# roseDwayane/EyeGaze-Multimodal

Measured on AMD Instinct MI355X. Metric: train samples/sec (gaze+EEG windows), higher is better.
Workload: dtype bf16; 1 GPU; cfg3: BASELINE configs[2]/[3]: + bidirectional cross-stream attention fusion; batch_per_gpu=256, global_batch=256, C=8, T=1024, seq_len=65, d_model=256, layers=6, step=fwd(train,dropout)+bwd+allreduce+clip+AdamW, parallelism=dp1

## Files before the change

### eyegaze_multimodal_amd/_lib.py

```python
from __future__ import annotations

import ctypes as C
from pathlib import Path

_PKG = Path(__file__).resolve().parent
LIB_PATH = _PKG / "libeyegaze_hip.so"

EG_F32, EG_BF16, EG_F16 = 0, 1, 2
ACT_NONE, ACT_RELU, ACT_GELU = 0, 1, 2
ABI_VERSION = 5


class EgError(RuntimeError):
    pass


class RowMap(C.Structure):
    _fields_ = [("row_stride", C.c_int64), ("group_stride", C.c_int64), ("rows_per_group", C.c_int32), ("_pad", C.c_int32)]


def rowmap(row_stride: int, group_stride: int = 0, rows_per_group: int = 0) -> RowMap:
    return RowMap(int(row_stride), int(group_stride), int(rows_per_group), 0)


# ... 19 lines not shown

class FfnDesc(C.Structure):
    _fields_ = [("A", C.c_void_p), ("W1", C.c_void_p), ("W2", C.c_void_p), ("H", C.c_void_p), ("C", C.c_void_p),
                ("bias1", C.c_void_p), ("bias2", C.c_void_p), ("gate", C.c_void_p), ("gate_bits_out", C.c_void_p),
                ("gate_bits_in", C.c_void_p), ("residual", C.c_void_p),
                ("state", C.c_void_p),
                ("lda", C.c_int64), ("ldh", C.c_int64), ("ldc", C.c_int64), ("ldg", C.c_int64), ("ldr", C.c_int64),
                ("M", C.c_int32), ("F", C.c_int32), ("act1", C.c_int32), ("dtype", C.c_int32),
                ("drop_h_p", C.c_float), ("drop_c1_p", C.c_float), ("drop_c2_p", C.c_float),
                ("drop_h_site", C.c_uint32), ("drop_c1_site", C.c_uint32), ("drop_c2_site", C.c_uint32),
                ("gate_scale", C.c_float),
                ("ln_gamma", C.c_void_p), ("ln_beta", C.c_void_p), ("ln_out", C.c_void_p), ("ln_stats", C.c_void_p)]


class LnBwdProjDesc(C.Structure):
    _fields_ = [("dy", C.c_void_p), ("x", C.c_void_p), ("stats", C.c_void_p), ("gamma", C.c_void_p), ("W_frag", C.c_void_p),
                ("dx", C.c_void_p), ("dx_drop", C.c_void_p), ("dC", C.c_void_p), ("partial", C.c_void_p), ("state", C.c_void_p),
                ("M", C.c_int32), ("d_model", C.c_int32), ("dtype", C.c_int32), ("partial_capacity_blocks", C.c_int32),
                ("drop1_p", C.c_float), ("drop2_p", C.c_float), ("drop1_site", C.c_uint32), ("drop2_site", C.c_uint32)]


class AttnBlockDesc(C.Structure):
    _fields_ = [("x", C.c_void_p), ("wqkv_frag", C.c_void_p), ("wo_frag", C.c_void_p), ("bqkv", C.c_void_p), ("bo", C.c_void_p),
                ("qkv", C.c_void_p), ("ctx", C.c_void_p), ("lse", C.c_void_p), ("r1", C.c_void_p), ("state", C.c_void_p),
                ("NB", C.c_int32), ("S", C.c_int32), ("d_model", C.c_int32), ("num_heads", C.c_int32), ("dtype", C.c_int32),
                ("attn_drop_p", C.c_float), ("out_drop_p", C.c_float), ("attn_drop_site", C.c_uint32), ("out_drop_site", C.c_uint32),
                ("ln_gamma", C.c_void_p), ("ln_beta", C.c_void_p), ("ln_out", C.c_void_p), ("ln_stats", C.c_void_p)]


class PackEntry(C.Structure):
    _fields_ = [("src", C.c_uint64), ("dst", C.c_uint64), ("rows", C.c_int32), ("cols", C.c_int32), ("ldd", C.c_int32),
                ("mode", C.c_int32), ("blk0", C.c_int32), ("nblk", C.c_int32)]


class PackEntryEx(C.Structure):
    _fields_ = [("src", C.c_uint64), ("dst", C.c_uint64), ("rows", C.c_int32), ("cols", C.c_int32), ("ldd", C.c_int32),
                ("mode", C.c_int32), ("blk0", C.c_int32), ("nblk", C.c_int32), ("p0", C.c_int32), ("p1", C.c_int32),
                ("p2", C.c_int32), ("p3", C.c_int32), ("src_elems", C.c_int64), ("dst_elems", C.c_int64)]


class TNProblem(C.Structure):
    _fields_ = [("dY", C.c_uint64), ("X", C.c_uint64), ("partial", C.c_uint64), ("ldy", C.c_int64), ("ldx", C.c_int64),
                ("N", C.c_int32), ("K", C.c_int32), ("part_rows", C.c_int32), ("has_bias", C.c_int32), ("blk0", C.c_int32),
                ("_pad", C.c_int32)]


class ReduceEntry(C.Structure):
    _fields_ = [("partial", C.c_uint64), ("out", C.c_uint64), ("n", C.c_int64), ("stride", C.c_int64),
                ("splits", C.c_int32), ("blk0", C.c_int32)]


class GemmTNDesc(C.Structure):
    _fields_ = [("dY", C.c_void_p), ("X", C.c_void_p), ("partial", C.c_void_p), ("y", RowMap), ("x", RowMap),
                ("M", C.c_int32), ("N", C.c_int32), ("K", C.c_int32), ("splits", C.c_int32), ("dtype", C.c_int32),
                ("x_tile_stride", C.c_int64), ("part_rows", C.c_int32), ("has_bias", C.c_int32), ("tile", C.c_int32)]


_P, _I, _L, _F, _U = C.c_void_p, C.c_int, C.c_int64, C.c_float, C.c_uint32

SIGNATURES = {
    "eg_device_info": [C.POINTER(C.c_int), C.c_char_p, _I],
    "eg_window_pack": [_P, _P, _I, _I, _I, _I, _I, _I, _I, _P],
    "eg_pack_table": [_P, _I, _I, _I, _P],
    "eg_pack_table_ex_check": [_P, _I, _I, C.POINTER(C.c_int)],
    "eg_pack_table_ex": [_P, _I, _I, _I, _P],
    "eg_cast": [_P, _P, _L, _I, _P],
    "eg_transpose_cast": [_P, _P, _I, _I, _I, _I, _P],
    "eg_pack_conv_weight": [_P, _P, _I, _I, _I, _I, _I, _I, _P],
    "eg_pack_convT_weight": [_P, _P, _I, _I, _I, _I, _I, _P],
    "eg_gemm_nt": [C.POINTER(GemmDesc), _P],
    "eg_gemm_nt_route": [C.POINTER(GemmDesc)],
    "eg_ffn_chain": [C.POINTER(FfnDesc), _P],
    "eg_ln_bwd_proj": [C.POINTER(LnBwdProjDesc), _P],
    "eg_ln_bwd_proj_blocks": [_I],
    "eg_attn_block_fwd": [C.POINTER(AttnBlockDesc), _P],
    "eg_attn_block_ok": [_I, _I, _I, _I],
    "eg_gemm_tn": [C.POINTER(GemmTNDesc), _P],
    "eg_reduce_partials": [_P, _P, _L, _I, _L, _I, _P],
    "eg_gemm_tn_grouped": [_P, _I, _I, _I, _I, _I, _P],
    "eg_gemm_tn_grouped256": [_P, _I, _I, _I, _I, _I, _P],
    "eg_reduce_table": [_P, _I, _I, _P],
    "eg_unpack_conv_wgrad": [_P, _P, _I, _I, _I, _I, _I, _I, _P],
    "eg_colsum": [_P, RowMap, _I, _I, _P, _I, _I, _P],
    "eg_layernorm_fwd": [_P, _P, _P, _P, _P, _I, _I, _I, _P],
    "eg_layernorm_bwd": [_P, _P, _P, _P, _P, _P, _P, _I, _I, _I, _I, _I, _F, _U, _F, _U, _P, _P],
    "eg_attention_fwd": [_P, _P, _P, _I, _I, _I, _I, _I, _F, _U, _P, _P],
    "eg_attention_bwd": [_P, _P, _P, _P, _P, _I, _I, _I, _I, _I, _F, _U, _P, _P],
    "eg_window_normalize": [_P, _P, _P, _I, _I, _I, _I, _P],
    "eg_attention_probs": [_P, _P, _P, _I, _I, _I, _I, _I, _P],
    "eg_attention_long_fwd": [_P, _P, _P, _I, _I, _I, _I, _I, _F, _U, _P, _P],
    "eg_attention_long_bwd": [_P, _P, _P, _P, _P, _I, _I, _I, _I, _I, _F, _U, _P, _P, _L, _P],
    "eg_attention_long_probs": [_P, _P, _P, _I, _I, _I, _I, _I, _P],
    "eg_rows_bcast_f32": [_P, _P, _P, _I, _I, _I, _I, _I, _I, _I, _P],
    "eg_rows_copy": [_P, _I, _I, _I, _I, _I, _I, _I, _I, _P],
    "eg_pool_fuse_fwd": [_P, _P, _P, _P, _P, _P, _P, _I, _I, _I, _I, _I, _I, _I, _P],
    "eg_pool_fuse_bwd": [_P, _P, _P, _P, _P, _P, _P, _P, _I, _I, _I, _I, _I, _I, _I, _P],
    "eg_classifier_ce_fwd": [_P, _P, _P, _P, _P, _P, _P, _I, _I, _I, _I, _P],
    "eg_classifier_ce_bwd": [_P, _P, _P, _P, _P, _P, _P, _P, _P, _P, _I, _I, _I, _I, _F, _I, _P],
    "eg_batch_rowsum": [_P, _P, _I, _I, _I, _I, _I, _P],
    "eg_rows_gather_gate": [_P, _P, _P, RowMap, _I, _I, _I, _I, _I, _I, _F, _I, _P],
    "eg_heads_fwd": [_P, _P, _P, _P, _P, _P, _P, _P, _P, _P, _P, _P, _P, _P, _I, _I, _I, _F, _U, _P, _I, _P],
    "eg_classifier_ce_bwd_fused": [_P, _P, _P, _P, _P, _P, _P, _P, _P, _P, _I, _I, _I, _I, _F, _I, _P],
    "eg_heads_bwd_chain": [_P, _P, _P, _P, _P, _P, _P, _P, _I, _I, _I, _P],
    "eg_heads_bwd_pool": [_P, _P, _P, _P, _P, _P, _P, _P, _P, _P, _P, _I, _I, _I, _I, _I, _I, _I, _P],
    "eg_token_grad_tail": [_P, _P, _P, RowMap, _P, _P, _I, _I, _I, _I, _I, _F, _I, _P],
    "eg_grad_sqnorm": [_P, _L, _P, _I, _P],
    "eg_grad_accumulate": [_P, _P, _L, _I, _P, _I, _P],
    "eg_clip_coef": [_P, _I, _F, _P, _P],
    "eg_grad_sqnorm_clip": [_P, _L, _P, _I, _F, _P, _P, _P],
    "eg_adamw": [_P, _P, _P, _P, _L, _F, _F, _F, _F, _P, _P],
    "eg_fill_f32": [_P, _L, _F, _P],
    "eg_adamw_group": [_P, _P, _P, _P, _L, _F, _F, _F, _F, _F, _P, _P],
    "eg_set_step_state": [_P, _U, _U, _F, _F, _F, _F, _I, _F, _I, _P],
    "eg_scaler_update": [_P, _F, _F, _I, _P],
    "eg_aux_symmetry": [_P, _P, _P, _P, _P, _I, _I, _P],
    "eg_aux_infonce": [_P, _P, _P, _F, _P, _P, _P, _P, _P, _I, _I, _P],
    "eg_aux_supcon": [_P, _P, _F, _P, _P, _P, _I, _I, _P],
    "eg_fuzzy_gate_fwd": [_P, _P, _P, _P, _P, _I, _I, _I, _F, _F, _F, _P],
    "eg_fusion_loop_loss": [_P, _P, _P, _P, _P, _P, _P, _P, _P, _P, _I, _I, _I, _F, _F, _F, _F, _F, _F, _P, _P],
    "eg_fuzzy_gate_bwd": [_P, _P, _P, _P, _P, _P, _P, _P, _I, _I, _I, _F, _F, _F, _P],
    "eg_ibs_analytic": [_P, _P, _P, _P, _P, _I, _I, _F, _I, _P, _P, _I, _P],
    "eg_ibs_pairs": [_P, _P, _P, _P, _P, _I, _I, _I, _F, _I, _P, _P, _I, _P],
    "eg_ibs_scalar": [_P, _P, _P, _P, _I, _I, _I, _F, _I, _P, _P, _I, _I, _I, _I, _P],
    "eg_affine_grad": [_P, _P, _P, _I, _I, _I, _I, _P],
    "eg_ibs_inorm": [_P, _P, _P, _P, _P, _P, _I, _I, _I, _I, _I, _I, _P],
    "eg_gelu_fwd": [_P, _P, _L, _I, _F, _U, _P, _P],
    "eg_gelu_bwd": [_P, _P, _P, _L, _I, _F, _U, _P, _P],
    "eg_stft_logmag": [_P, _P, _P, _I, _I, _I, _I, _I, _P],
    "eg_spec_conv1_fwd": [_P, _P, _P, _P, _I, _I, _I, _I, _P],
    "eg_spec_conv1_bwd": [_P, _P, _P, _P, _P, _I, _I, _I, _I, _P],
    "eg_spec_avgpool_fwd": [_P, _P, _I, _I, _I, _I, _P],
    "eg_spec_avgpool_bwd": [_P, _P, _P, _I, _I, _I, _I, _P],
    "eg_pack_conv2d_weight": [_P, _P, _I, _I, _I, _I, _P],
    "eg_unpack_conv2d_wgrad": [_P, _P, _I, _I, _I, _P],
    "eg_conv2d_wgrad_flat": [_P, _P, _P, _P, _L, _L, _I, _I, _I, _P],
    "eg_conv2d_wgrad_flat_splits": [_L, _I],
    "eg_conv2d_flat": [_P, _P, _P, _P, _L, _L, _I, _I, _I, _I, _I, _I, _I, _P],
}
_lib = None


def lib() -> C.CDLL:
    global _lib
    if _lib is not None:
        return _lib
    if not LIB_PATH.exists():
        raise EgError(f"{LIB_PATH} is missing: build it with `python -m eyegaze_multimodal_amd.build` "
                      "(hipcc --offload-arch=gfx950).  There is no CPU fallback.")
    l = C.CDLL(str(LIB_PATH))
    l.eg_abi_version.restype = C.c_int
    if l.eg_abi_version() != ABI_VERSION:
        raise EgError(f"ABI mismatch: library {l.eg_abi_version()} vs binding {ABI_VERSION}")
    l.eg_last_error.restype = C.c_char_p
    for name, args in SIGNATURES.items():
        fn = getattr(l, name, None)
        if fn is None:
            continue
        fn.argtypes = args
        fn.restype = C.c_int
    _lib = l
    return l


def gate_bits_bytes(M: int, F: int) -> int:
    l = lib()
    l.eg_ffn_gate_bits_bytes.restype = C.c_int64
# ... 24 lines not shown
```

### eyegaze_multimodal_amd/build.py

```python
from __future__ import annotations

import os
import subprocess
import sys
from concurrent.futures import ThreadPoolExecutor
from pathlib import Path

PKG = Path(__file__).resolve().parent
CSRC = PKG / "csrc"
LIB = PKG / "libeyegaze_hip.so"
SOURCES = ["prep.hip", "gemm.hip", "rsgemm.hip", "widegemm.hip", "ffn.hip", "lnproj.hip", "attnblock.hip", "norm.hip", "attention.hip", "attention_long.hip", "heads.hip", "optim.hip", "signal.hip", "spec.hip", "aux.hip"]
HIPCC = os.environ.get("HIPCC", "/opt/rocm/bin/hipcc")
FLAGS = ["--offload-arch=gfx950", "-O3", "-fPIC", "-std=c++17", "-Wno-unused-result"]


def _stale(obj: Path, src: Path) -> bool:
    if not obj.exists():
        return True
    deps = [src, CSRC / "common.h", PKG.parent / "include" / "eyegaze_hip.h"]
    return any(d.stat().st_mtime > obj.stat().st_mtime for d in deps)


def build(force: bool = False, verbose: bool = True) -> Path:
    srcs = [CSRC / s for s in SOURCES if (CSRC / s).exists()]
    objs = [CSRC / (s.stem + ".o") for s in srcs]

    def cc(pair):
        src, obj = pair
        if force or _stale(obj, src):
            cmd = [HIPCC, *FLAGS, "-c", str(src), "-o", str(obj)]
            if verbose:
                print(" ".join(cmd), flush=True)
            subprocess.run(cmd, check=True)
            return True
        return False

    with ThreadPoolExecutor(max_workers=min(6, len(srcs))) as ex:
        rebuilt = list(ex.map(cc, zip(srcs, objs)))
    if any(rebuilt) or not LIB.exists() or force:
        cmd = [HIPCC, "--offload-arch=gfx950", "-shared", "-fPIC", "-o", str(LIB), *map(str, objs)]
        if verbose:
            print(" ".join(cmd), flush=True)
        subprocess.run(cmd, check=True)
    return LIB


if __name__ == "__main__":
    build(force="--force" in sys.argv)
    print(LIB)
```

### eyegaze_multimodal_amd/engine.py

```python
from __future__ import annotations

import ctypes as C
import math
import os
from typing import Dict, List, Optional, Tuple

import torch

from . import _lib as L
from ._lib import EG_BF16, EG_F16, EG_F32, GemmDesc, GemmTNDesc, StepState, call, ptr, rowmap

SITE_CONV0, SITE_CONV1, SITE_SPEC, SITE_IBSTOK, SITE_IBSGEN, SITE_CLS, SITE_IBSCLS = 1, 2, 3, 4, 5, 6, 7


def scramble_seed(seed: int) -> int:
    m = (1 << 64) - 1
    z = (seed + 0x9E3779B97F4A7C15) & m
    z = ((z ^ (z >> 30)) * 0xBF58476D1CE4E5B9) & m
    z = ((z ^ (z >> 27)) * 0x94D049BB133111EB) & m
    return z ^ (z >> 31)


def _reduce_blocks(n: int, splits: int) -> int:
    cols = n // 4
# ... 71 lines not shown
        if self.acc is None:
            self.acc = torch.zeros_like(self.grad)
        return self.acc

    def p_ptr(self, name: str) -> int:
        return self.flat.data_ptr() + 4 * self.offsets[name]

    def g_ptr(self, name: str) -> int:
        return self.grad.data_ptr() + 4 * self.offsets[name]

    def grad_view(self, name: str, p: torch.nn.Parameter) -> torch.Tensor:
        o = self.offsets[name]
        return self.grad[o:o + p.numel()].view(p.shape)

    def has(self, name: str) -> bool:
        return name in self.offsets


class Engine:
    LN_PARTIAL_BLOCKS = 2048
    SQ_BLOCKS = 1024

    def __init__(self, model, B: int, T: int, device: torch.device, dtype: int, state_dev: Optional[torch.Tensor] = None):
        cfg = model.cfg
        self._shared_state = state_dev
        self.model, self.cfg, self.B, self.T, self.device, self.dtype = model, cfg, B, T, device, dtype
        self.tdtype = {EG_BF16: torch.bfloat16, EG_F16: torch.float16, EG_F32: torch.float32}[dtype]
        self.es = 4 if dtype == EG_F32 else 2
        self.bk = 32 if dtype == EG_F32 else 64
        self.scaler_on = dtype == EG_F16 and os.environ.get("EYEGAZE_LOSS_SCALING", "1") != "0"
        self.scaler_cfg = dict(init_scale=65536.0, growth=2.0, backoff=0.5, growth_interval=2000)
        d, H = cfg.d_model, cfg.num_heads
        if d % H != 0 or d // H != 32:
            raise L.EgError(f"HIP attention core needs d_model/num_heads == 32 (got {d}/{H})")
        if cfg.conv_layers != 2:
            raise L.EgError("HIP path implements the reference's 2-layer temporal conv front-end (conv_layers=2)")
        if d % 64 != 0 or cfg.d_ff % 64 != 0:
            raise L.EgError("d_model and d_ff must be multiples of 64")
        k, s = cfg.conv_kernel_size, cfg.conv_stride
        pad = k // 2
        self.k, self.s, self.pad = k, s, pad
        self.NB = 2 * B
        self.C = cfg.in_channels
        self.Cp = _align(self.C, 8)
        self.T1 = (T + 2 * pad - k) // s + 1
        self.T2 = (self.T1 + 2 * pad - k) // s + 1
        self.J = (k + s - 1) // s
        self.K0 = _align(k * self.Cp, self.bk)
        self.Tp = _align(max(T + 2 * pad, s * (self.T1 - 1) + self.K0 // self.Cp + 1), 8)
        self.U = (self.T1 + 2 * pad + s - 1) // s
        self.R0 = self.U * s
        self.RY = self.T2 + 2 * (self.J - 1)
        self.n_ibs = cfg.num_ibs_tokens
        self.n_spec = self.C if cfg.use_spectrogram else 0
        self.off = 1 + self.n_ibs + self.n_spec
        self.S = sequence_length(cfg, T)
        self.attn_long = self.S > ATTN_SHORT_MAX_S
        self.M = self.NB * self.S
        self._want_attn_block = os.environ.get("EYEGAZE_ATTN_BLOCK", "1") != "0"
        self.fp: FlatParams = model._flat
        self.stream = 0
        self.probes = {}
        self.cus = torch.cuda.get_device_properties(device).multi_processor_count if device.type == "cuda" else 256
        self.attn_block = False
        self.fuse_ffn = (dtype != EG_F32 and cfg.d_model == 256 and cfg.d_ff % 128 == 0
                         and os.environ.get("EYEGAZE_FFN", "1") != "0")
        env_nb = os.environ.get("EYEGAZE_LN_BLOCKS")
        trips = max(1, self.M // 8192)
        self.LN_BLOCKS = int(env_nb) if env_nb else min(self.LN_PARTIAL_BLOCKS, 4 * self.cus,
                                                        max(1, (self.M + 8 * trips - 1) // (8 * trips)))
        if not 1 <= self.LN_BLOCKS <= self.LN_PARTIAL_BLOCKS:
            raise L.EgError(f"EYEGAZE_LN_BLOCKS={env_nb} is outside [1, {self.LN_PARTIAL_BLOCKS}] (rows of the LayerNorm-backward "
                            "partial buffer)")
        self.ln_nblk_cap = max(self.LN_BLOCKS, (self.M + 63) // 64)
        self.probe_all = None
        self.attn_block = bool(self._want_attn_block and dtype != EG_F32
                               and L.lib().eg_attn_block_ok(self.S, cfg.d_model, cfg.num_heads, dtype))
        self.ln_fuse = os.environ.get("EYEGAZE_LN_FUSE", "1") != "0"
        self.ln_proj = (dtype != EG_F32 and cfg.d_model == 256 and os.environ.get("EYEGAZE_LN_PROJ", "1") != "0")
        self.ln_proj_blocks = L.lib().eg_ln_bwd_proj_blocks(self.M) if self.ln_proj else 0
        self.fused_tail = dtype != EG_F32
        self.pack_unused = False
        self.fused_norm_clip = False
        self._alloc()
        self.packed_version = -1
        self._recording = False
        self._plan = []
        self._acc_norm_ready = False

    def _t(self, *shape, dtype=None):
        return torch.zeros(*shape, device=self.device, dtype=dtype or self.tdtype)

    def _alloc(self):
        cfg, d, F, L_ = self.cfg, self.cfg.d_model, self.cfg.d_ff, self.cfg.num_layers
        NB, M, S, H, B = self.NB, self.M, self.S, self.cfg.num_heads, self.B
        f32 = torch.float32
        w = {}
        w["conv0"] = self._t(d, self.K0)
        w["conv1"] = self._t(d, self.k * d)
        w["conv1T"] = self._t(self.s, d, self.J * d)
        w["pos"] = self._t(cfg.max_len, d)
        for l in list(range(L_)) + (["x"] if cfg.use_cross_attention else []):
            w[f"qkv{l}"] = self._t(3 * d, d)
            w[f"qkvT{l}"] = self._t(d, 3 * d)
            w[f"o{l}"] = self._t(d, d)
            w[f"oT{l}"] = self._t(d, d)
            w[f"bqkv{l}"] = self._t(3 * d, dtype=f32)
            if self.ln_proj and l != "x":
                w[f"oTf{l}"] = self._t(d * d)
            if self.attn_block and l != "x":
                w[f"wqkvb{l}"] = self._t(3 * d * d)
                w[f"wob{l}"] = self._t(d * d)
            if l != "x":
                w[f"w1{l}"] = self._t(F, d)
                w[f"w1T{l}"] = self._t(d, F)
                w[f"w2{l}"] = self._t(d, F)
                w[f"w2T{l}"] = self._t(F, d)
                if self.fuse_ffn:
                    for nm in ("w1f", "w2f", "w2Tf", "w1Tf"):
                        w[f"{nm}{l}"] = self._t(F * d)
        w["sf"] = self._t(d, 3 * d)
        w["sfT"] = self._t(3 * d, d)
        w["c0"] = self._t(d, 3 * d)
        w["c0T"] = self._t(3 * d, d)
        if cfg.use_ibs:
            w["i0"] = self._t(d // 2, d)
            w["i0T"] = self._t(d, _align(d // 2, self.bk))
        self.w = w
        a = {}
        a["xt"] = self._t(NB, self.Tp, self.Cp)
        a["h0pad"] = self._t(NB, self.R0, d)
        a["h1"] = self._t(NB * self.T2, d)
        a["x0"] = self._t(M, d)
        for l in range(L_):
            a[f"qkv{l}"] = self._t(M, 3 * d)
            a[f"lse{l}"] = self._t(NB, H, S, dtype=f32)
            a[f"ctx{l}"] = self._t(M, d)
            a[f"r1_{l}"] = self._t(M, d)
            a[f"st1_{l}"] = self._t(M, 2, dtype=f32)
            a[f"y1_{l}"] = self._t(M, d)
            a[f"hff{l}"] = self._t(M, F)
            if self.fuse_ffn:
                a[f"gbits{l}"] = torch.zeros(L.gate_bits_bytes(M, F) // 8, device=self.device, dtype=torch.int64)
            a[f"r2_{l}"] = self._t(M, d)
            a[f"st2_{l}"] = self._t(M, 2, dtype=f32)
            a[f"x{l + 1}"] = self._t(M, d)
        a["stf"] = self._t(M, 2, dtype=f32)
        a["zn"] = self._t(M, d)
        if cfg.use_cross_attention:
            a["qkvx"] = self._t(M, 3 * d)
            a["lsex"] = self._t(NB, H, S, dtype=f32)
            a["ctxx"] = self._t(M, d)
            a["rx"] = self._t(M, d)
            a["stx"] = self._t(M, 2, dtype=f32)
            a["zc"] = self._t(M, d)
        a["cls1"] = self._t(B, d, dtype=f32)
        a["cls2"] = self._t(B, d, dtype=f32)
        a["comb"] = self._t(B, 3 * d)
        a["zf"] = self._t(B, 3 * d)
        a["hcl"] = self._t(B, d)
        a["logits"] = self._t(B, cfg.num_classes, dtype=f32)
        a["sloss"] = self._t(B, dtype=f32)
        a["loss"] = self._t(1, dtype=f32)
        a["heads_ctr"] = torch.zeros(1, device=self.device, dtype=torch.int32)
        if cfg.use_ibs:
            a["ibs_pool_f"] = self._t(B, d, dtype=f32)
# ... 740 lines not shown
            attn_block_bwd("cross_attn.cross_attn.", "x", a["zn"], drx, drm, B, xs["attn"], other,
                           g["dqkv_x"] if gx else g["dqkv"], gx)
            dz, other = other, dz
            if not gx:
                seg("cross")
        self.ln_bwd(dz, a[f"x{Lr}"], a["stf"], "encoder.norm", other, slot=nslot("encoder.norm"))
        dz, other = other, dz
        seg("encoder.norm")
        for l in reversed(range(Lr)):
            pre, sites = f"encoder.layers.{l}.", _layer_sites(l)
            dYf = g[f"dYf{l}"] if grouped else (g["drm"] if has_drop else g["dr"])
            dYo = g[f"dYo{l}"] if grouped else (g["drm"] if has_drop else g["dr"])
            dh = g[f"dh{l}"] if grouped else g["dh"]
            dqkv = g[f"dqkv{l}"] if grouped else g["dqkv"]
            s2 = self._ln_slot[pre + "ln2"] if grouped else None
            s1 = self._ln_slot[pre + "ln1"] if grouped else None
            if has_drop:
                self.ln_bwd(dz, a[f"r2_{l}"], a[f"st2_{l}"], pre + "ln2", g["dr"], dYf, d1=(p, sites["ffn_b"]),
                            d2=(p, sites["drop2"]), slot=s2)
            else:
                self.ln_bwd(dz, a[f"r2_{l}"], a[f"st2_{l}"], pre + "ln2", dYf, None, slot=s2)
            dr = g["dr"] if has_drop else dYf
            if not grouped:
                self.wgrad(ptr(dYf), ptr(a[f"hff{l}"]), 0, M, d, F, linear=[pre + "ffn.linear2"])
            if self.fuse_ffn:
                self.ffn(ptr(dYf), ptr(w[f"w2Tf{l}"]), ptr(w[f"w1Tf{l}"]), ptr(dh), ptr(g["dy1"]), M, F, residual=ptr(dr),
                         bits_in=ptr(a[f"gbits{l}"]), gate_scale=sc)
            else:
                self.gemm(ptr(dYf), ptr(w[f"w2T{l}"]), ptr(dh), M, F, d, gate=ptr(a[f"hff{l}"]), gate_scale=sc)
            if not grouped:
                self.wgrad(ptr(dh), ptr(a[f"y1_{l}"]), 0, M, F, d, linear=[pre + "ffn.linear1"])
            if not self.fuse_ffn:
                self.gemm(ptr(dh), ptr(w[f"w1T{l}"]), ptr(g["dy1"]), M, d, F, residual=ptr(dr))
            if self.ln_proj:
                self.ln_bwd_proj(g["dy1"], a[f"r1_{l}"], a[f"st1_{l}"], pre + "ln1", w[f"oTf{l}"], g["dr"], dYo, g["dctx"],
                                 d1=(p, sites["drop1"]) if has_drop else (0.0, 0), slot=s1)
                dr = g["dr"]
            else:
                if has_drop:
                    self.ln_bwd(g["dy1"], a[f"r1_{l}"], a[f"st1_{l}"], pre + "ln1", g["dr"], dYo, d1=(p, sites["drop1"]), slot=s1)
                else:
                    self.ln_bwd(g["dy1"], a[f"r1_{l}"], a[f"st1_{l}"], pre + "ln1", dYo, None, slot=s1)
                dr = g["dr"] if has_drop else dYo
            attn_block_bwd(pre + "mha.", l, a[f"x{l}"], dr, dYo, 0, sites["attn"], other, dqkv, grouped, dctx_done=self.ln_proj)
            dz, other = other, dz
            if not grouped:
                seg(f"layer{l}")
            elif pieced and l == self._wg_plan["split_layer"]:
                self._wgrad_group_launch(self._wg_plan["pieces"][0])
                if gx:
                    seg("cross")
                for ll in reversed(self._wg_plan["pieces"][0]["layers"]):
                    seg(f"layer{ll}")
        if grouped:
            if pieced:
                self._wgrad_group_launch(self._wg_plan["pieces"][1])
                for ll in reversed(self._wg_plan["pieces"][1]["layers"]):
                    seg(f"layer{ll}")
            else:
                self._wgrad_group_launch(self._wg_plan["whole_norms"] if defer_norms else None)
                if gx:
                    seg("cross")
                for l in reversed(range(Lr)):
                    seg(f"layer{l}")
        dseq = dz
        ymap = rowmap(d, self.RY * d, self.T2)
        fused_tokens = bool(self.fused_tail) and self.dtype != EG_F32 and d % 64 == 0
        if fused_tokens:
            call("eg_token_grad_tail", ptr(dseq), ptr(a["h1"]), ptr(g["dy1pad"]) + (self.J - 1) * d * es, ymap,
                 fp.g_ptr("pos_embed.pos_embed.weight"), fp.g_ptr("cls_token"), NB, S, d, self.T2, self.off, sc01, self.dtype, st)
        else:
            call("eg_batch_rowsum", ptr(dseq), fp.g_ptr("pos_embed.pos_embed.weight"), NB, S, d, S, self.dtype, st)
            call("eg_cast", fp.g_ptr("pos_embed.pos_embed.weight"), fp.g_ptr("cls_token"), d, EG_F32, st)
        self.model._extra_tokens_bwd(self, dseq)
        seg("tokens")
        if not fused_tokens:
            call("eg_rows_gather_gate", ptr(dseq), ptr(a["h1"]), ptr(g["dy1pad"]) + (self.J - 1) * d * es, ymap, NB, S, d,
                 self.T2, self.off, 0, sc01, self.dtype, st)
        dy1 = ptr(g["dy1pad"]) + (self.J - 1) * d * es
        self.wgrad(dy1, ptr(a["h0pad"]), fp.g_ptr("temporal_conv.convs.1.weight"), NB * self.T2, d, self.k * d, y=ymap,
                   x=rowmap(self.s * d, self.R0 * d, self.T2), out_b=fp.g_ptr("temporal_conv.convs.1.bias"),
                   conv=(d, self.k, d))
        seg("conv1")
        for ph in range(self.s):
            self.gemm(ptr(g["dy1pad"]), ptr(w["conv1T"]) + ph * d * self.J * d * es, ptr(g["dh0pad"]) + ph * d * es,
                      NB * self.U, d, self.J * d, a=rowmap(d, self.RY * d, self.U), c=rowmap(self.s * d, self.R0 * d, self.U),
                      gate=ptr(a["h0pad"]) + ph * d * es, gate_scale=sc01)
        h0map = rowmap(d, self.R0 * d, self.T1)
        self.wgrad(ptr(g["dh0pad"]) + self.pad * d * es, ptr(a["xt"]), fp.g_ptr("temporal_conv.convs.0.weight"),
                   NB * self.T1, d, self.K0, y=h0map, x=rowmap(self.s * self.Cp, self.Tp * self.Cp, self.T1),
                   out_b=fp.g_ptr("temporal_conv.convs.0.bias"), conv=(self.C, self.k, self.Cp))
        seg("frontend")

    def bucket_ranges(self) -> Dict[str, Tuple[int, int]]:
        key = self.fp.grad.data_ptr()
        if getattr(self, "_ranges_key", None) != key:
            from .ddp import bucket_ranges
            fp = self.fp
            self._ranges = bucket_ranges(fp.names, fp.offsets, fp.total, self.cfg.num_layers, self.cfg.use_cross_attention)
            self._ranges_key = key
        return self._ranges

    def accumulate(self, first: bool, segment: Optional[str] = None, norm: bool = False) -> torch.Tensor:
        self._alloc_bwd()
        self.stream = self._cur_stream()
        acc = self.fp.accumulator()
        if segment is None:
            b, e = 0, self.fp.total
        else:
            rg = self.bucket_ranges()
            if segment not in rg:
                raise L.EgError(f"accumulate: no gradient bucket named {segment!r} (have {sorted(rg)})")
            b, e = rg[segment]
            if norm:
                raise L.EgError("accumulate: the fused norm partials cover the whole buffer, not one bucket")
        sq = 0
        if norm:
            if "sqpart" not in self.g:
                self.g["sqpart"] = self._t(self.SQ_BLOCKS, dtype=torch.float32)
            sq = ptr(self.g["sqpart"])
        self._acc_norm_ready = False
        if e > b:
            call("eg_grad_accumulate", ptr(acc) + 4 * b, ptr(self.fp.grad) + 4 * b, e - b, int(bool(first)), sq,
                 self.SQ_BLOCKS if norm else 0, self.stream)
        self._acc_norm_ready = bool(norm)
        return acc

    def optimizer_step(self, m: torch.Tensor, v: torch.Tensor, max_norm: float = 1.0, betas=(0.9, 0.999), eps=1e-8,
                       weight_decay=0.01, accumulated: bool = False, norm_ready: bool = False):
        self._alloc_bwd()
        self.stream = self._cur_stream()
        nblk = self.SQ_BLOCKS
        if "sqpart" not in self.g:
            self.g["sqpart"] = self._t(nblk, dtype=torch.float32)
        if accumulated and self.fp.acc is None:
            raise L.EgError("optimizer_step(accumulated=True) without a preceding Engine.accumulate")
        if norm_ready and not (accumulated and self._acc_norm_ready):
            raise L.EgError("optimizer_step(norm_ready=True): no norm partials of the whole accumulator from this engine")
        grad = self.fp.acc if accumulated else self.fp.grad
        self._acc_norm_ready = False
        if norm_ready or not self.fused_norm_clip:
            if not norm_ready:
                call("eg_grad_sqnorm", ptr(grad), self.fp.total, ptr(self.g["sqpart"]), nblk, self.stream)
            call("eg_clip_coef", ptr(self.g["sqpart"]), nblk, max_norm, self.st_ptr, self.stream)
        else:
            if "sq_ctr" not in self.g:
                self.g["sq_ctr"] = torch.zeros(1, device=self.device, dtype=torch.int32)
            call("eg_grad_sqnorm_clip", ptr(grad), self.fp.total, ptr(self.g["sqpart"]), nblk, max_norm, self.st_ptr,
                 ptr(self.g["sq_ctr"]), self.stream)
        call("eg_adamw", ptr(self.fp.flat), ptr(grad), ptr(m), ptr(v), self.fp.total, betas[0], betas[1], eps,
             weight_decay, self.st_ptr, self.stream)
        if self.scaler_on:
            c = self.scaler_cfg
            call("eg_scaler_update", self.st_ptr, c["growth"], c["backoff"], c["growth_interval"], self.stream)
```

### include/eyegaze_hip.h

```cpp
#ifndef EYEGAZE_HIP_H
#define EYEGAZE_HIP_H

#include <stdint.h>

#ifdef __cplusplus
extern "C" {
#endif

#define EG_ABI_VERSION 5
enum { EG_F32 = 0, EG_BF16 = 1, EG_F16 = 2 };
enum { EG_ACT_NONE = 0, EG_ACT_RELU = 1, EG_ACT_GELU = 2 };

int eg_abi_version(void);
const char* eg_last_error(void);
int eg_device_info(int* cu_count, char* arch, int arch_len);

typedef struct eg_step_state {
  uint32_t seed_lo, seed_hi;
  float lr;
  float bias_corr1;
  float bias_corr2;
  float grad_scale;
  float clip_coef;
  float grad_norm;
// ... 79 lines not shown
  float drop_h_p, drop_c1_p, drop_c2_p;
  uint32_t drop_h_site, drop_c1_site, drop_c2_site;
  float gate_scale;
  const float* ln_gamma;
  const float* ln_beta;
  void* ln_out;
  float* ln_stats;
} eg_ffn_desc;
int eg_ffn_chain(const eg_ffn_desc* d, void* stream);
int64_t eg_ffn_gate_bits_bytes(int M, int F);

typedef struct eg_ln_bwd_proj_desc {
  const void* dy;
  const void* x;
  const float* stats;
  const float* gamma;
  const void* W_frag;
  void* dx;
  void* dx_drop;
  void* dC;
  float* partial;
  const eg_step_state* state;
  int32_t M, d_model, dtype, partial_capacity_blocks;
  float drop1_p, drop2_p;
  uint32_t drop1_site, drop2_site;
} eg_ln_bwd_proj_desc;
int eg_ln_bwd_proj(const eg_ln_bwd_proj_desc* d, void* stream);
int eg_ln_bwd_proj_blocks(int M);

typedef struct eg_attn_block_desc {
  const void* x;
  const void* wqkv_frag;
  const void* wo_frag;
  const float* bqkv;
  const float* bo;
  void* qkv;
  void* ctx;
  float* lse;
  void* r1;
  const eg_step_state* state;
  int32_t NB, S, d_model, num_heads, dtype;
  float attn_drop_p, out_drop_p;
  uint32_t attn_drop_site, out_drop_site;
  const float* ln_gamma;
  const float* ln_beta;
  void* ln_out;
  float* ln_stats;
} eg_attn_block_desc;
int eg_attn_block_fwd(const eg_attn_block_desc* d, void* stream);
int eg_attn_block_ok(int S, int d_model, int num_heads, int dtype);

typedef struct eg_gemm_tn_desc {
  const void* dY;
  const void* X;
  float* partial;
  eg_rowmap y, x;
  int32_t M, N, K, splits;
  int32_t dtype;
  int64_t x_tile_stride;
  int32_t part_rows;
  int32_t has_bias;
  int32_t tile;
} eg_gemm_tn_desc;
int eg_gemm_tn(const eg_gemm_tn_desc* d, void* stream);
typedef struct eg_tn_problem {
  uint64_t dY, X, partial;
  int64_t ldy, ldx;
  int32_t N, K, part_rows, has_bias, blk0, _pad;
} eg_tn_problem;
#define EG_REDUCE_WIDE_SPLITS 8
typedef struct eg_reduce_entry {
  uint64_t partial, out;
  int64_t n, stride;
  int32_t splits, blk0;
} eg_reduce_entry;
int eg_gemm_tn_grouped(const eg_tn_problem* probs, int nprob, int total_blocks, int M, int splits, int dtype, void* stream);
int eg_gemm_tn_grouped256(const eg_tn_problem* probs, int nprob, int total_blocks, int M, int splits, int dtype, void* stream);
int eg_reduce_table(const eg_reduce_entry* table, int nentries, int total_blocks, void* stream);
int eg_reduce_partials(float* partial, float* out, int64_t n, int splits, int64_t split_stride, int accumulate,
                       void* stream);
int eg_unpack_conv_wgrad(const float* partial, float* dW, int splits, int N, int Cin, int k, int Cp, int Kp,
                         void* stream);
int eg_colsum(const void* Y, eg_rowmap y, int M, int N, float* partial, int nblk, int dtype, void* stream);

int eg_layernorm_fwd(const void* x, const float* gamma, const float* beta, void* y, float* stats, int M, int D,
                     int dtype, void* stream);
int eg_layernorm_bwd(const void* dy, const void* x, const float* stats, const float* gamma, void* dx, void* dx_drop,
                     float* partial, int nblk, int partial_capacity_blocks, int M, int D, int dtype, float drop1_p,
                     uint32_t drop1_site, float drop2_p, uint32_t drop2_site, const eg_step_state* state, void* stream);

int eg_attention_fwd(const void* qkv, void* ctx, float* lse, int NB, int S, int H, int kv_shift, int dtype,
                     float drop_p, uint32_t drop_site, const eg_step_state* state, void* stream);
int eg_attention_bwd(const void* qkv, const void* ctx, const void* dctx, const float* lse, void* dqkv, int NB, int S,
                     int H, int kv_shift, int dtype, float drop_p, uint32_t drop_site, const eg_step_state* state,
                     void* stream);
int eg_attention_probs(const void* qkv, const float* lse, float* probs, int NB, int S, int H, int kv_shift, int dtype,
                       void* stream);

#define EG_ATTN_LONG_MAX_S 2048
int eg_attention_long_fwd(const void* qkv, void* ctx, float* lse, int NB, int S, int H, int kv_shift, int dtype,
                          float drop_p, uint32_t drop_site, const eg_step_state* state, void* stream);
int eg_attention_long_bwd(const void* qkv, const void* ctx, const void* dctx, const float* lse, void* dqkv, int NB, int S,
                          int H, int kv_shift, int dtype, float drop_p, uint32_t drop_site, const eg_step_state* state,
                          float* scratch, int64_t scratch_elems, void* stream);
int eg_attention_long_probs(const void* qkv, const float* lse, float* probs, int NB, int S, int H, int kv_shift, int dtype,
                            void* stream);

int eg_rows_bcast_f32(const float* src, const float* pos, void* seq, int NB, int S, int D, int R, int off, int src_nb,
                      int dtype, void* stream);
int eg_rows_copy(void* seq, int S, int D, int R, int off, int b_src0, int b_dst0, int nb, int dtype, void* stream);
int eg_pool_fuse_fwd(const void* z, float* cls1, float* cls2, void* comb, void* zf, float* ibs_pool_f, void* ibs_pool,
                     int B, int S, int D, int off, int n_ibs, int ibs_first, int dtype, void* stream);
int eg_pool_fuse_bwd(const void* z, const void* dcomb, const void* dzf, const float* gcls1, const float* gcls2,
                     const void* dibs_pool, const float* gibs_pool, void* dz, int B, int S, int D, int off, int n_ibs,
                     int ibs_first, int dtype, void* stream);
int eg_classifier_ce_fwd(const void* h, const float* W, const float* bias, const int64_t* labels, float* logits,
                         float* sample_loss, float* loss, int B, int K, int ncls, int dtype, void* stream);
int eg_classifier_ce_bwd(const void* h, const float* W, const float* logits, const int64_t* labels, const float* gloss,
                         const float* glogits, float* dlogits, void* dh, float* dW, float* db, int B, int K, int ncls,
                         int use_gate, float gate_scale, int dtype, void* stream);
int eg_batch_rowsum(const void* dseq, float* out, int NB, int S, int D, int rows, int dtype, void* stream);
int eg_rows_gather_gate(const void* src, const void* gate, void* dst, eg_rowmap dmap, int nb, int S, int D, int R,
                        int off, int pair_shift, float gate_scale, int dtype, void* stream);

int eg_heads_fwd(const void* comb, void* zf, void* hcl, const void* Wsf, const float* bsf, const void* Wc0, const float* bc0,
                 const float* W3, const float* b3, const int64_t* labels, float* logits, float* sample_loss, float* loss,
                 uint32_t* counter, int B, int D, int ncls, float drop_p, uint32_t drop_site, const eg_step_state* state,
                 int dtype, void* stream);
int eg_classifier_ce_bwd_fused(const void* h, const float* W, const float* logits, const int64_t* labels, const float* gloss,
                               const float* glogits, float* dlogits, void* dh, float* dW, float* db, int B, int K, int ncls,
                               int use_gate, float gate_scale, int dtype, void* stream);
int eg_heads_bwd_chain(const void* dhcl, const void* c0T, const void* sfT, const void* zf, void* dzf, void* dcomb, float* dWc0,
                       float* dbc0, int B, int D, int dtype, void* stream);
int eg_heads_bwd_pool(const void* z, const void* dcomb, const void* dzf, const float* gcls1, const float* gcls2,
                      const void* dibs_pool, const float* gibs_pool, void* dz, const void* comb, float* dWsf, float* dbsf, int B,
                      int S, int D, int off, int n_ibs, int ibs_first, int dtype, void* stream);
int eg_token_grad_tail(const void* dseq, const void* gate, void* dst, eg_rowmap dmap, float* pos_grad, float* cls_grad, int NB,
                       int S, int D, int R, int off, float gate_scale, int dtype, void* stream);

int eg_aux_symmetry(const float* cls1, const float* cls2, float* loss, float* d_cls1, float* d_cls2, int B, int D, void* stream);
int eg_aux_infonce(const float* ibs, const float* cls1, const float* cls2, float temperature, float* loss, float* d_ibs,
                   float* d_cls1, float* d_cls2, float* work, int B, int D, void* stream);
int eg_aux_supcon(const float* ibs, const int64_t* labels, float temperature, float* loss, float* d_ibs, float* work, int B,
                  int D, void* stream);

int eg_fusion_loop_loss(const float* fused, const float* z_img, const float* z_eeg, const int64_t* labels, const float* params,
                        float* losses, float* dfused, float* daux_img, float* daux_eeg, float* dtau, int B, int K, int mode,
                        float eps_temp, float lambda_aux_img, float lambda_aux_eeg, float lambda_reg, float t_min, float t_max,
                        const eg_step_state* state, void* stream);
int eg_fuzzy_gate_fwd(const float* z_img, const float* z_eeg, const float* params, float* fused, float* alpha, int B,
                      int K, int mode, float eps_temp, float eps_log, float eps_div, void* stream);
int eg_fuzzy_gate_bwd(const float* z_img, const float* z_eeg, const float* params, const float* dfused, const float* dalpha,
                      float* dz_img, float* dz_eeg, float* partial, int B, int K, int mode, float eps_temp, float eps_log,
                      float eps_div, void* stream);

int eg_grad_sqnorm(const float* g, int64_t n, float* partial, int nblk, void* stream);
int eg_grad_accumulate(float* acc, const float* g, int64_t n, int first, float* sq_partial, int nblk, void* stream);
int eg_clip_coef(const float* partial, int nblk, float max_norm, eg_step_state* state, void* stream);
int eg_grad_sqnorm_clip(const float* g, int64_t n, float* partial, int nblk, float max_norm, eg_step_state* state,
                        uint32_t* counter, void* stream);
int eg_adamw(float* p, const float* g, float* m, float* v, int64_t n, float beta1, float beta2, float eps,
             float weight_decay, const eg_step_state* state, void* stream);
int eg_fill_f32(float* p, int64_t n, float value, void* stream);
int eg_adamw_group(float* p, const float* g, float* m, float* v, int64_t n, float beta1, float beta2, float eps,
                   float weight_decay, float lr_mult, const eg_step_state* state, void* stream);
int eg_scaler_update(eg_step_state* state, float growth, float backoff, int growth_interval, void* stream);
// ... 37 lines not shown
```

Baseline: 83070 samples/s.

## Add dedicated conv0 weight-gradient kernel and skip zero taps in conv1 dgrad

Adds a specialized HIP kernel for the first temporal conv's weight gradient. It stages a 64-row dY tile plus the overlapping strided X window in LDS, uses transposed LDS reads feeding MFMA, writes split-K partials, and finishes with a reduce-and-unpack kernel. The bias gradient uses colsum plus a partial reduce. Separately, the conv1 input-gradient GEMMs now skip the leading taps that are all zero for each phase, which shortens K. This adds two or three extra launches and a new code path gated by a stride/span check, falling back to the generic wgrad when that check fails.

New measurement: 83560 samples/s (median of 6 runs). Within noise of the previous version (+0.6%).

```diff
diff --git a/eyegaze_multimodal_amd/_lib.py b/eyegaze_multimodal_amd/_lib.py
--- a/eyegaze_multimodal_amd/_lib.py
+++ b/eyegaze_multimodal_amd/_lib.py
@@ -125,6 +125,9 @@
     "eg_reduce_table": [_P, _I, _I, _P],
     "eg_unpack_conv_wgrad": [_P, _P, _I, _I, _I, _I, _I, _I, _P],
     "eg_colsum": [_P, RowMap, _I, _I, _P, _I, _I, _P],
+    "eg_conv0_wgrad_ok": [RowMap, _I, _I, _I],
+    "eg_conv0_wgrad_splits": [_I, _I],
+    "eg_conv0_wgrad": [_P, _P, RowMap, RowMap, _I, _I, _I, _I, _I, _I, _P, _L, _P, _I, _P],
     "eg_layernorm_fwd": [_P, _P, _P, _P, _P, _I, _I, _I, _P],
     "eg_layernorm_bwd": [_P, _P, _P, _P, _P, _P, _P, _I, _I, _I, _I, _I, _F, _U, _F, _U, _P, _P],
     "eg_attention_fwd": [_P, _P, _P, _I, _I, _I, _I, _I, _F, _U, _P, _P],
diff --git a/eyegaze_multimodal_amd/build.py b/eyegaze_multimodal_amd/build.py
--- a/eyegaze_multimodal_amd/build.py
+++ b/eyegaze_multimodal_amd/build.py
@@ -9,7 +9,7 @@
 PKG = Path(__file__).resolve().parent
 CSRC = PKG / "csrc"
 LIB = PKG / "libeyegaze_hip.so"
-SOURCES = ["prep.hip", "gemm.hip", "rsgemm.hip", "widegemm.hip", "ffn.hip", "lnproj.hip", "attnblock.hip", "norm.hip", "attention.hip", "attention_long.hip", "heads.hip", "optim.hip", "signal.hip", "spec.hip", "aux.hip"]
+SOURCES = ["prep.hip", "gemm.hip", "rsgemm.hip", "widegemm.hip", "conv0.hip", "ffn.hip", "lnproj.hip", "attnblock.hip", "norm.hip", "attention.hip", "attention_long.hip", "heads.hip", "optim.hip", "signal.hip", "spec.hip", "aux.hip"]
 HIPCC = os.environ.get("HIPCC", "/opt/rocm/bin/hipcc")
 FLAGS = ["--offload-arch=gfx950", "-O3", "-fPIC", "-std=c++17", "-Wno-unused-result"]
 
diff --git a/eyegaze_multimodal_amd/csrc/conv0.hip b/eyegaze_multimodal_amd/csrc/conv0.hip
--- /dev/null
+++ b/eyegaze_multimodal_amd/csrc/conv0.hip
@@ -0,0 +1,238 @@
+#include "common.h"
+
+namespace {
+
+constexpr int C0_K = 256;
+constexpr int C0_NS = 64;
+constexpr int C0_RS = 64;
+constexpr int C0_YTILE = C0_RS * 256;
+constexpr int C0_XCH = 3;
+constexpr int C0_XBYTES = C0_XCH * 256 * 16;
+constexpr int C0_LDS = C0_YTILE + C0_XBYTES;
+constexpr int C0_OCC = 3;
+
+template <typename T>
+struct Conv0Wgrad {
+  const T* dY; const T* X; float* partial;
+  RowMap y, x;
+  int M, N, Kl, splits, rows_per_split, slices;
+};
+
+__device__ __forceinline__ int c0_swz(int r) { return (((r & 3) | ((r >> 1) & 4)) << 1); }
+
+template <typename T>
+__device__ __forceinline__ void c0_mma(const char* bufY, const char* bufX, const int (&xr)[2], int k0, int nk, int lane,
+                                       f32x4 (&acc)[4][4]) {
+  const int g = lane >> 4, q = (lane & 15) >> 2, pp = lane & 3;
+  typedef typename H16<T>::frag frag;
+  typedef __attribute__((ext_vector_type(8))) short s16x8;
+  frag yf[4], xf[4];
+#pragma unroll
+  for (int i = 0; i < 4; ++i) {
+    s16x4 lo[2];
+#pragma unroll
+    for (int h = 0; h < 2; ++h) {
+      const int r = 8 * g + 4 * h + q;
+      const int cy = i * 16 + 4 * pp;
+      const int ay = r * 256 + (((cy >> 3) ^ c0_swz(r)) << 4) + ((cy >> 2) & 1) * 8;
+      lo[h] = __builtin_amdgcn_ds_read_tr16_b64_v4i16((s16x4 __attribute__((address_space(3)))*)(bufY + ay));
+    }
+    s16x8 ty = {lo[0][0], lo[0][1], lo[0][2], lo[0][3], lo[1][0], lo[1][1], lo[1][2], lo[1][3]};
+    yf[i] = __builtin_bit_cast(frag, ty);
+  }
+#pragma unroll
+  for (int i = 0; i < 4; ++i)
+    if (i < nk) {
+      s16x4 hi[2];
+#pragma unroll
+      for (int h = 0; h < 2; ++h)
+        hi[h] = __builtin_amdgcn_ds_read_tr16_b64_v4i16(
+            (s16x4 __attribute__((address_space(3)))*)(bufX + xr[h] + (k0 + i * 16 + 4 * pp) * 2));
+      s16x8 tx = {hi[0][0], hi[0][1], hi[0][2], hi[0][3], hi[1][0], hi[1][1], hi[1][2], hi[1][3]};
+      xf[i] = __builtin_bit_cast(frag, tx);
+    }
+#pragma unroll
+  for (int ki = 0; ki < 4; ++ki)
+    if (ki < nk) {
+#pragma unroll
+      for (int ni = 0; ni < 4; ++ni) acc[ki][ni] = H16<T>::mfma(xf[ki], yf[ni], acc[ki][ni]);
+    }
+}
+
+template <typename T>
+__global__ __launch_bounds__(256, C0_OCC) void conv0_wgrad_kernel(Conv0Wgrad<T> p) {
+  extern __shared__ __attribute__((aligned(16))) char smem[];
+  char* const bufY = smem;
+  char* const bufX = smem + C0_YTILE;
+  const int tid = threadIdx.x, lane = tid & 63, wave = tid >> 6;
+  const int bid = xcd_remap(blockIdx.x, gridDim.x);
+  const int split = bid / p.slices, n0 = (bid % p.slices) * C0_NS;
+  const int mbeg = split * p.rows_per_split;
+  const int mend = min(p.M, mbeg + p.rows_per_split);
+  const int k0 = wave * 64;
+  const int nk = min(4, max(0, (p.Kl - k0) >> 4));
+
+  f32x4 acc[4][4];
+#pragma unroll
+  for (int i = 0; i < 4; ++i)
+#pragma unroll
+    for (int j = 0; j < 4; ++j) acc[i][j] = (f32x4){0.f, 0.f, 0.f, 0.f};
+
+  constexpr int YCH = C0_RS * 8 / 256;
+  u32x4 ry[YCH], rx[C0_XCH];
+  auto load_tile = [&](int mt) {
+    const u32x4 z = {0u, 0u, 0u, 0u};
+#pragma unroll
+    for (int i = 0; i < YCH; ++i) {
+      const int c = tid + 256 * i;
+      const int m = mt + (c >> 3);
+      ry[i] = m < mend ? *(const u32x4*)(p.dY + row_off(p.y, m) + n0 + (c & 7) * 8) : z;
+    }
+    const long long xb = row_off(p.x, mt);
+    const int nch = (int)((row_off(p.x, min(mt + C0_RS, mend) - 1) - xb + C0_K) >> 3);
+#pragma unroll
+    for (int i = 0; i < C0_XCH; ++i) {
+      const int c = tid + 256 * i;
+      rx[i] = c < nch ? *(const u32x4*)(p.X + xb + c * 8) : z;
+    }
+  };
+  auto store_tile = [&]() {
+#pragma unroll
+    for (int i = 0; i < YCH; ++i) {
+      const int c = tid + 256 * i;
+      const int row = c >> 3, ch = c & 7;
+      *(u32x4*)(bufY + row * 256 + ((ch ^ c0_swz(row)) << 4)) = ry[i];
+    }
+#pragma unroll
+    for (int i = 0; i < C0_XCH; ++i) *(u32x4*)(bufX + (tid + 256 * i) * 16) = rx[i];
+  };
+  const int nt = (mend - mbeg + C0_RS - 1) / C0_RS;
+  const int lr = 8 * (lane >> 4) + ((lane & 15) >> 2);
+  if (nt > 0) load_tile(mbeg);
+  for (int it = 0; it < nt; ++it) {
+    const int mt = mbeg + it * C0_RS;
+    store_tile();
+    __syncthreads();
+    if (it + 1 < nt) load_tile(mt + C0_RS);
+    const long long xb = row_off(p.x, mt);
+#pragma unroll
+    for (int sub = 0; sub < C0_RS / 32; ++sub) {
+      int xr[2];
+#pragma unroll
+      for (int h = 0; h < 2; ++h) xr[h] = (int)(row_off(p.x, min(mt + sub * 32 + lr + 4 * h, mend - 1)) - xb) * 2;
+      c0_mma<T>(bufY + sub * 32 * 256, bufX, xr, k0, nk, lane, acc);
+    }
+    __syncthreads();
+  }
+  float* out = p.partial + (size_t)split * p.N * p.Kl;
+  const int l15 = lane & 15, g = lane >> 4;
+#pragma unroll
+  for (int ki = 0; ki < 4; ++ki)
+#pragma unroll
+    for (int ni = 0; ni < 4; ++ni) {
+      const int n = n0 + ni * 16 + l15;
+      const int k = k0 + ki * 16 + 4 * g;
+      if (k < p.Kl) *(f32x4*)(out + (size_t)n * p.Kl + k) = acc[ki][ni];
+    }
+}
+
+__global__ __launch_bounds__(64) void conv0_wgrad_finish_kernel(const float* __restrict__ partial, float* __restrict__ dW,
+                                                                int splits, int N, int Kl, int Cin, int k, int Cp) {
+  __shared__ float row[C0_K];
+  const int n = blockIdx.x, c4 = threadIdx.x;
+  const size_t slab = (size_t)N * Kl;
+  if (c4 * 4 < Kl) {
+    const float* src = partial + (size_t)n * Kl + c4 * 4;
+    f32x4 s = *(const f32x4*)src;
+    int sp = 1;
+    for (; sp + 8 <= splits; sp += 8) {
+      f32x4 a[8];
+#pragma unroll
+      for (int j = 0; j < 8; ++j) a[j] = *(const f32x4*)(src + (size_t)(sp + j) * slab);
+#pragma unroll
+      for (int j = 0; j < 8; ++j) s += a[j];
+    }
+    for (; sp < splits; ++sp) s += *(const f32x4*)(src + (size_t)sp * slab);
+#pragma unroll
+    for (int e = 0; e < 4; ++e) {
+      const int kk = c4 * 4 + e, tap = kk / Cp, c = kk - tap * Cp;
+      if (tap < k && c < Cin) row[c * k + tap] = s[e];
+    }
+  }
+  __syncthreads();
+  float* dst = dW + (size_t)n * Cin * k;
+  for (int j = c4; j < Cin * k; j += 64) dst[j] = row[j];
+}
+
+template <typename T>
+static int launch_conv0_wgrad(const void* dY, const void* X, const eg_rowmap& y, const eg_rowmap& x, int M, int N, int Kl,
+                              int splits, float* partial, hipStream_t s) {
+  Conv0Wgrad<T> p;
+  p.dY = (const T*)dY; p.X = (const T*)X; p.partial = partial;
+  p.y = to_rowmap(y); p.x = to_rowmap(x);
+  p.M = M; p.N = N; p.Kl = Kl; p.splits = splits; p.slices = N / C0_NS;
+  p.rows_per_split = ((M + splits - 1) / splits + C0_RS - 1) / C0_RS * C0_RS;
+  hipLaunchKernelGGL(conv0_wgrad_kernel<T>, dim3(p.slices * splits), dim3(256), C0_LDS, s, p);
+  EG_LAUNCH_CHECK("conv0_wgrad");
+  return 0;
+}
+
+}
+
+static long long c0_worst_span(const eg_rowmap& x) {
+  if (x.row_stride < 0) return -1;
+  long long span = (long long)(C0_RS - 1) * x.row_stride + C0_K;
+  if (x.rows_per_group > 0) {
+    const long long gap = x.group_stride - (long long)x.rows_per_group * x.row_stride;
+    if (gap < 0) return -1;
+    span += (long long)((C0_RS - 1 + x.rows_per_group - 1) / x.rows_per_group) * gap;
+  }
+  return span;
+}
+
+extern "C" int eg_conv0_wgrad_ok(eg_rowmap x, int N, int K, int dtype) {
+  if (dtype != EG_BF16 && dtype != EG_F16) return 0;
+  if (N <= 0 || N % C0_NS != 0 || K != C0_K) return 0;
+  if (x.row_stride % 8 != 0 || x.group_stride % 8 != 0) return 0;
+  const long long span = c0_worst_span(x);
+  return span > 0 && span * 2 <= C0_XBYTES ? 1 : 0;
+}
+
+extern "C" int eg_conv0_wgrad_splits(int M, int N) {
+  if (M <= 0 || N <= 0 || N % C0_NS != 0) return 0;
+  const int tiles = ((N + 127) / 128) * (C0_K / 128);
+  const int by_rows = (M + 127) / 128, by_grid = 768 / tiles > 0 ? 768 / tiles : 1;
+  const int s = by_rows < by_grid ? by_rows : by_grid;
+  return s < 1 ? 1 : s;
+}
+
+extern "C" int eg_conv0_wgrad(const void* dY, const void* X, eg_rowmap y, eg_rowmap x, int M, int N, int K, int Cin, int k,
+                              int Cp, float* partial, int64_t partial_floats, float* dW, int dtype, void* stream) {
+  EG_CHECK(dY && X && partial && dW, "eg_conv0_wgrad: null operand");
+  EG_CHECK(dtype == EG_BF16 || dtype == EG_F16, "eg_conv0_wgrad: 16-bit dtypes only (got %d)", dtype);
+  EG_CHECK(M > 0 && N > 0 && N % C0_NS == 0 && K == C0_K, "eg_conv0_wgrad: needs N %% 64 == 0 and K == 256 (M=%d N=%d K=%d)", M, N, K);
+  EG_CHECK(Cin > 0 && k > 0 && Cp >= Cin && k * Cp <= K, "eg_conv0_wgrad: bad convolution Cin=%d k=%d Cp=%d", Cin, k, Cp);
+  EG_CHECK(y.row_stride % 8 == 0 && y.group_stride % 8 == 0 && x.row_stride % 8 == 0 && x.group_stride % 8 == 0,
+           "eg_conv0_wgrad: rows must be 16-B aligned");
+  EG_CHECK(((uintptr_t)dY | (uintptr_t)X | (uintptr_t)partial | (uintptr_t)dW) % 16 == 0, "eg_conv0_wgrad: alignment");
+  EG_CHECK(eg_conv0_wgrad_ok(x, N, K, dtype), "eg_conv0_wgrad: %d consecutive X rows (stride %lld, %d per group of stride %lld) "
+           "span more than the %d bytes the kernel stages", C0_RS, (long long)x.row_stride, x.rows_per_group,
+           (long long)x.group_stride, C0_XBYTES);
+  const int splits = eg_conv0_wgrad_splits(M, N);
+  const int Kl = (k * Cp + 15) / 16 * 16;
+  EG_CHECK(partial_floats >= (int64_t)splits * N * Kl, "eg_conv0_wgrad: the partial buffer holds %lld floats, %lld needed",
+           (long long)partial_floats, (long long)splits * N * Kl);
+  hipStream_t s = (hipStream_t)stream;
+  static bool attr = false;
+  if (!attr) {
+    (void)hipFuncSetAttribute((const void*)conv0_wgrad_kernel<bf16_t>, hipFuncAttributeMaxDynamicSharedMemorySize, C0_LDS);
+    (void)hipFuncSetAttribute((const void*)conv0_wgrad_kernel<f16_t>, hipFuncAttributeMaxDynamicSharedMemorySize, C0_LDS);
+    attr = true;
+  }
+  const int rc = dtype == EG_BF16 ? launch_conv0_wgrad<bf16_t>(dY, X, y, x, M, N, Kl, splits, partial, s)
+                                  : launch_conv0_wgrad<f16_t>(dY, X, y, x, M, N, Kl, splits, partial, s);
+  if (rc) return rc;
+  hipLaunchKernelGGL(conv0_wgrad_finish_kernel, dim3(N), dim3(64), 0, s, partial, dW, splits, N, Kl, Cin, k, Cp);
+  EG_LAUNCH_CHECK("conv0_wgrad_finish");
+  return 0;
+}
diff --git a/eyegaze_multimodal_amd/engine.py b/eyegaze_multimodal_amd/engine.py
--- a/eyegaze_multimodal_amd/engine.py
+++ b/eyegaze_multimodal_amd/engine.py
@@ -177,6 +177,7 @@
         self.fused_tail = dtype != EG_F32
         self.pack_unused = False
         self.fused_norm_clip = False
+        self.conv0_native = bool(L.lib().eg_conv0_wgrad_ok(rowmap(self.s * self.Cp, self.Tp * self.Cp, self.T1), d, self.K0, dtype))
         self._alloc()
         self.packed_version = -1
         self._recording = False
@@ -1083,15 +1084,33 @@
                    x=rowmap(self.s * d, self.R0 * d, self.T2), out_b=fp.g_ptr("temporal_conv.convs.1.bias"),
                    conv=(d, self.k, d))
         seg("conv1")
+        self.conv1_dgrad(sc01)
+        self.conv0_wgrad()
+        seg("frontend")
+
+    def conv1_dgrad(self, sc01: float, skip_zero_taps: bool = True):
+        d, es, NB, a, g, w = self.cfg.d_model, self.es, self.NB, self.a, self.g, self.w
         for ph in range(self.s):
-            self.gemm(ptr(g["dy1pad"]), ptr(w["conv1T"]) + ph * d * self.J * d * es, ptr(g["dh0pad"]) + ph * d * es,
-                      NB * self.U, d, self.J * d, a=rowmap(d, self.RY * d, self.U), c=rowmap(self.s * d, self.R0 * d, self.U),
+            live = (self.k - ph + self.s - 1) // self.s
+            z = self.J - live if skip_zero_taps else 0
+            self.gemm(ptr(g["dy1pad"]) + z * d * es, ptr(w["conv1T"]) + (ph * d * self.J * d + z * d) * es,
+                      ptr(g["dh0pad"]) + ph * d * es, NB * self.U, d, (self.J - z) * d, ldw=self.J * d,
+                      a=rowmap(d, self.RY * d, self.U), c=rowmap(self.s * d, self.R0 * d, self.U),
                       gate=ptr(a["h0pad"]) + ph * d * es, gate_scale=sc01)
-        h0map = rowmap(d, self.R0 * d, self.T1)
-        self.wgrad(ptr(g["dh0pad"]) + self.pad * d * es, ptr(a["xt"]), fp.g_ptr("temporal_conv.convs.0.weight"),
-                   NB * self.T1, d, self.K0, y=h0map, x=rowmap(self.s * self.Cp, self.Tp * self.Cp, self.T1),
-                   out_b=fp.g_ptr("temporal_conv.convs.0.bias"), conv=(self.C, self.k, self.Cp))
-        seg("frontend")
+
+    def conv0_wgrad(self):
+        d, es, fp, g, a = self.cfg.d_model, self.es, self.fp, self.g, self.a
+        dY, M = ptr(g["dh0pad"]) + self.pad * d * es, self.NB * self.T1
+        h0map, xmap = rowmap(d, self.R0 * d, self.T1), rowmap(self.s * self.Cp, self.Tp * self.Cp, self.T1)
+        out_w, out_b = fp.g_ptr("temporal_conv.convs.0.weight"), fp.g_ptr("temporal_conv.convs.0.bias")
+        if self.conv0_native:
+            call("eg_conv0_wgrad", dY, ptr(a["xt"]), h0map, xmap, M, d, self.K0, self.C, self.k, self.Cp, ptr(g["partial"]),
+                 self.tn_cap, out_w, self.dtype, self.stream)
+            nblk = min(512, (M + 63) // 64)
+            call("eg_colsum", dY, h0map, M, d, ptr(g["cspart"]), nblk, self.dtype, self.stream)
+            call("eg_reduce_partials", ptr(g["cspart"]), out_b, d, nblk, d, 0, self.stream)
+        else:
+            self.wgrad(dY, ptr(a["xt"]), out_w, M, d, self.K0, y=h0map, x=xmap, out_b=out_b, conv=(self.C, self.k, self.Cp))
 
     def bucket_ranges(self) -> Dict[str, Tuple[int, int]]:
         key = self.fp.grad.data_ptr()
diff --git a/include/eyegaze_hip.h b/include/eyegaze_hip.h
--- a/include/eyegaze_hip.h
+++ b/include/eyegaze_hip.h
@@ -185,6 +185,10 @@
 int eg_unpack_conv_wgrad(const float* partial, float* dW, int splits, int N, int Cin, int k, int Cp, int Kp,
                          void* stream);
 int eg_colsum(const void* Y, eg_rowmap y, int M, int N, float* partial, int nblk, int dtype, void* stream);
+int eg_conv0_wgrad_ok(eg_rowmap x, int N, int K, int dtype);
+int eg_conv0_wgrad_splits(int M, int N);
+int eg_conv0_wgrad(const void* dY, const void* X, eg_rowmap y, eg_rowmap x, int M, int N, int K, int Cin, int k, int Cp,
+                   float* partial, int64_t partial_floats, float* dW, int dtype, void* stream);
 
 int eg_layernorm_fwd(const void* x, const float* gamma, const float* beta, void* y, float* stats, int M, int D,
                      int dtype, void* stream);
```
